# ChaoLiangTHU/rec_now

Measured on AMD Instinct MI355X. Metric: samples/sec fwd+bwd, in-batch pairwise + DCN-v2, B=65536 at 1/2/4/8 GPUs, higher is better.
Workload: dtype f32 via 3 x bf16 six-term split (bf16 MFMA, f32 accumulate; per-product error <= 2^-25)

## Files before the change

rec_now_amd/csrc/gemm_shortk.hip:

```cpp
#include "gemm_split.hpp"

#define SK_BM 128
#define SK_BN 128
#define SK_BK 16

#ifndef RN_SK_PLAIN
#define SK_LDS4(ptr) __builtin_nontemporal_load(reinterpret_cast<const f32x4*>(ptr))
#define SK_STS4(ptr, v) __builtin_nontemporal_store((v), reinterpret_cast<f32x4*>(ptr))
#else
#define SK_LDS4(ptr) (*reinterpret_cast<const f32x4*>(ptr))
#define SK_STS4(ptr, v) (*reinterpret_cast<f32x4*>(ptr) = (v))
#endif
__host__ __device__ constexpr int sk_wg_per_cu(int EP, int DUAL, bool PRE, int NK = 0, bool SPL = false) {
    if (SPL) return 2;
    return (DUAL >= 4 || PRE || (NK > 0 && DUAL == 2)) ? 2 : (EP == 3 || DUAL == 2 || DUAL == 3 || NK > 0) ? 3 : 4;
}

template <bool B_KC, int EP, int DUAL, bool PRE = false, int NK = 0, bool SPL = false>
__global__ void __launch_bounds__(GEMM_THREADS, sk_wg_per_cu(EP, DUAL, PRE, NK, SPL))
k_gemm_shortk(const GemmK p, int row_tiles, int col_tiles, int xcd_aware, const char* __restrict__ b_planes, int64_t b_plane_bytes) {
    static_assert(!SPL || NK >= 3, "split precision: the ring schedule only");
    static_assert(!PRE || ((EP == 1 || EP == 2) && DUAL != 2 && DUAL != 4), "whole-tile prefetch: emul (EP 1) or the old C (EP 2)");
    static_assert(NK % 3 == 0, "ring schedule: three register sets, the same set holds k-tile 0 of every tile");
    static_assert(!PRE || NK == 0 || NK >= 7, "ring schedule: the four groups of the emul tile go out at k-tiles 0, 2, 4, 6");
    using TA = Tile<SK_BM, SK_BK, true>;
    using TB = Tile<SK_BN, SK_BK, B_KC>;
    constexpr int A_SZ = SK_BK * TA::LD, B_SZ = SK_BK * TB::LD, BUF = SPL ? SPL_STAGE / 4 : A_SZ + B_SZ;
    static_assert(4 * 16 * 36 <= BUF, "half sub-tile staging of 4 waves fits one operand buffer");
    extern __shared__ __attribute__((aligned(16))) float smem[];
    const int lane = threadIdx.x & 63, wave = threadIdx.x >> 6;
    const int wm = wave >> 1, wn = wave & 1;
    const int a_off = (lane >> 5) * TA::LD + wm * 64 + (lane & 31);
    const int b_off = (lane >> 5) * TB::LD + wn * 64 + (lane & 31);
    const int col_l = lane & 31, row_l = 4 * (lane >> 5);
    const int rr0 = lane >> 3, cc = (lane & 7) * 4;
    const unsigned e_lane = (unsigned)((wm * 64 + rr0) * p.lde + wn * 64 + cc);
    const unsigned c_lane = (unsigned)((wm * 64 + rr0) * p.ldc + wn * 64 + cc);
    const unsigned f_lane = (unsigned)((wm * 64 + rr0) * p.lde2 + wn * 64 + cc);
    const unsigned d_lane = (unsigned)((wm * 64 + rr0) * p.ldc2 + wn * 64 + cc);
    const unsigned g_lane = (unsigned)((wm * 64 + rr0) * p.lde3 + wn * 64 + cc);
    const int nk = p.K / SK_BK;
    const int ntiles = row_tiles * col_tiles;
    constexpr bool EARLY = NK >= 3 && ((EP && !PRE) || DUAL == 2 || DUAL == 4);
    constexpr bool ONCE = DUAL == 5 || DUAL == 6;
    static_assert(!ONCE || (EP == 0 && NK >= 3), "the one-go input gradient: ring schedule, no emul / accumulate");

    auto tile_of = [&](int slot, int& m0, int& n0) {
        int rt, ct;
        if (xcd_aware) {
            const int xcd = slot & 7, idx = slot >> 3;
            rt = (idx / col_tiles) * 8 + xcd;
            ct = idx % col_tiles;
        } else {
            rt = slot / col_tiles;
            ct = slot % col_tiles;
        }
        m0 = rt * SK_BM;
        n0 = ct * SK_BN;
    };

    TA ta;
    TB tb;
    ta.init(p.lda);
    tb.init(p.ldb);
    int slot = blockIdx.x;
    if (slot >= ntiles) return;
    int m0, n0;
    tile_of(slot, m0, n0);
    f32x4 ra[NK ? 3 : 1][TA::NV], rb[(NK && !SPL) ? 3 : 1][TB::NV];
    u32x4 rp[SPL ? 3 : 1][3];
    unsigned sa_bo = (unsigned)(((threadIdx.x >> 1) * p.lda + 8 * (threadIdx.x & 1)) * 4);
    unsigned sb_bo = (unsigned)((((threadIdx.x >> 7) * p.N) + (threadIdx.x & 127)) * 16);
    const int sa_soff = ((threadIdx.x & 1) * SPL_PLANE_H + (threadIdx.x >> 1)) * 16;
    const int sb_soff = SPL_OPER + ((threadIdx.x >> 7) * SPL_PLANE_H + (threadIdx.x & 127)) * 16;
    const int sfa_off = ((lane >> 5) * SPL_PLANE_H + wm * 64 + (lane & 31)) * 16;
    const int sfb_off = SPL_OPER + ((lane >> 5) * SPL_PLANE_H + wn * 64 + (lane & 31)) * 16;
    auto ring_load = [&](int set, int mm, int nn, int k0) {
        if constexpr (SPL) {
            const char* __restrict__ pa = reinterpret_cast<const char*>(p.A + (int64_t)mm * p.lda + k0);
            const char* __restrict__ pb = b_planes + ((int64_t)(k0 >> 3) * p.N + nn) * 16;
            asm volatile("" : "+v"(sa_bo));
            ra[set][0] = *reinterpret_cast<const f32x4*>(pa + sa_bo);
            ra[set][1] = *reinterpret_cast<const f32x4*>(pa + sa_bo + 16);
            asm volatile("" : "+v"(sb_bo));
#pragma unroll
            for (int q = 0; q < 3; ++q) rp[SPL ? set : 0][q] = *reinterpret_cast<const u32x4*>(pb + q * b_plane_bytes + sb_bo);
        } else {
        const char* __restrict__ pa = reinterpret_cast<const char*>(p.A + TA::tile_base(p.lda, mm, k0));
        const char* __restrict__ pb = reinterpret_cast<const char*>(p.B + TB::tile_base(p.ldb, nn, k0));
#pragma unroll
        for (int i = 0; i < TA::NV; ++i) {
            asm volatile("" : "+v"(ta.boff[i]));
            ra[set][i] = *reinterpret_cast<const f32x4*>(pa + ta.boff[i]);
        }
#pragma unroll
        for (int i = 0; i < TB::NV; ++i) {
            asm volatile("" : "+v"(tb.boff[i]));
            rb[SPL ? 0 : set][i] = *reinterpret_cast<const f32x4*>(pb + tb.boff[i]);
        }
        }
    };
    auto ring_store = [&](int set, float* S) {
        if constexpr (SPL) {
            char* Sc = reinterpret_cast<char*>(S);
            const float x[8] = {ra[set][0].x, ra[set][0].y, ra[set][0].z, ra[set][0].w, ra[set][1].x, ra[set][1].y, ra[set][1].z, ra[set][1].w};
            u32x4 w[3];
            spl_split8(x, w);
#pragma unroll
            for (int q = 0; q < 3; ++q) *reinterpret_cast<u32x4*>(Sc + sa_soff + q * SPL_PLANE) = w[q];
#pragma unroll
            for (int q = 0; q < 3; ++q) *reinterpret_cast<u32x4*>(Sc + sb_soff + q * SPL_PLANE) = rp[SPL ? set : 0][q];
        } else {
#pragma unroll
        for (int i = 0; i < TA::NV; ++i) { ta.v[i] = ra[set][i]; ta.store_slot(i, S); }
#pragma unroll
        for (int i = 0; i < TB::NV; ++i) { tb.v[i] = rb[SPL ? 0 : set][i]; tb.store_slot(i, S + A_SZ); }
        }
    };
    if (NK) {
        ring_load(0, m0, n0, 0);
        ring_load(1, m0, n0, SK_BK);
        ring_store(0, smem);
    } else {
        ta.template load_fast<false>(p.A, nullptr, 0, 0, p.lda, m0, 0);
        tb.template load_fast<false>(p.B, nullptr, 0, 0, p.ldb, n0, 0);
        ta.store(smem);
        tb.store(smem + A_SZ);
    }
    __syncthreads();
    int f = 0;
    for (; slot < ntiles; slot += gridDim.x) {
        const int nslot = slot + gridDim.x;
        const bool has_next = nslot < ntiles;
        int m0n = NK ? m0 : 0, n0n = NK ? n0 : 0;
        if (has_next) tile_of(nslot, m0n, n0n);
#ifdef RN_GEMM_TRACE
#define SK_TR(i) do { if (p.trace && threadIdx.x == 0) p.trace[(long long)slot * 8 + (i)] = wall_clock64(); } while (0)
        if (p.trace && threadIdx.x == 0) {
            p.trace[(long long)slot * 8 + 5] = clock64();
            p.trace[(long long)slot * 8 + 4] = __builtin_amdgcn_s_getreg((4) | (0 << 6) | ((32 - 1) << 11)) |
                                               ((long long)__builtin_amdgcn_s_getreg((20) | (0 << 6) | ((4 - 1) << 11)) << 32);
        }
#else
#define SK_TR(i) do { } while (0)
#endif
        SK_TR(0); SK_TR(1);
        if (p.prio == 1) __builtin_amdgcn_s_setprio(1);
        else if (p.prio == 2) __builtin_amdgcn_s_setprio(2);
        else if (p.prio == 3) __builtin_amdgcn_s_setprio(3);
        f32x16 acc[2][2];
#pragma unroll
        for (int i = 0; i < 2; ++i)
#pragma unroll
            for (int j = 0; j < 2; ++j)
#pragma unroll
                for (int r = 0; r < 16; ++r) acc[i][j][r] = 0.f;
        f32x4 evt[PRE ? 4 : 1][4];
        const float* Etp = !PRE ? nullptr : EP == 1 ? p.emul + (int64_t)m0 * p.lde + n0 : p.C + (int64_t)m0 * p.ldc + n0;
        const int64_t ldp = EP == 1 ? p.lde : p.ldc;
        auto pre_load = [&](int s2) {
#pragma unroll
            for (int q = 0; q < 4; ++q)
                evt[PRE ? s2 : 0][q] = SK_LDS4(Etp + (int64_t)((s2 >> 1) * 32 + q * 8) * ldp + (s2 & 1) * 32 + (EP == 1 ? e_lane : c_lane));
        };
        auto ktile = [&](int cur, int npairs, int nset = -1, float* Sn = nullptr) {
            if constexpr (SPL) {
                const char* S = reinterpret_cast<const char*>(smem + cur * BUF);
                char* Sc = reinterpret_cast<char*>(Sn);
                bf16x8 af[3][2], bf[3][2];
#pragma unroll
                for (int q = 0; q < 3; ++q)
#pragma unroll
                    for (int i = 0; i < 2; ++i) {
                        af[q][i] = *reinterpret_cast<const bf16x8*>(S + q * SPL_PLANE + sfa_off + i * 512);
                        bf[q][i] = *reinterpret_cast<const bf16x8*>(S + q * SPL_PLANE + sfb_off + i * 512);
                    }
                u32x4 w[3];
                const int ns = nset < 0 ? 0 : nset;
                auto pairs = [&](int e0) {
                    const float x[4] = {e0 ? ra[ns][1].x : ra[ns][0].x, e0 ? ra[ns][1].y : ra[ns][0].y, e0 ? ra[ns][1].z : ra[ns][0].z, e0 ? ra[ns][1].w : ra[ns][0].w};
#pragma unroll
                    for (int e = 0; e < 2; ++e) {
                        unsigned p1, p2, p3;
                        spl_split2(x[2 * e], x[2 * e + 1], p1, p2, p3);
                        w[0][e0 + e] = p1; w[1][e0 + e] = p2; w[2][e0 + e] = p3;
                    }
                };
                __builtin_amdgcn_sched_barrier(0);
#define SKS_TERM(SA, SB)                                                                                              \
                _Pragma("unroll") for (int i = 0; i < 2; ++i)                                                         \
                    _Pragma("unroll") for (int j = 0; j < 2; ++j)                                                     \
                        acc[i][j] = __builtin_amdgcn_mfma_f32_32x32x16_bf16(af[SA][i], bf[SB][j], acc[i][j], 0, 0, 0);
                SKS_TERM(0, 0)
                if (nset >= 0) pairs(0);
                __builtin_amdgcn_sched_barrier(0);
                SKS_TERM(0, 1)
                if (nset >= 0) pairs(2);
                __builtin_amdgcn_sched_barrier(0);
                SKS_TERM(1, 0)
                if (nset >= 0) {
#pragma unroll
                    for (int q = 0; q < 3; ++q) *reinterpret_cast<u32x4*>(Sc + sa_soff + q * SPL_PLANE) = w[q];
                }
                __builtin_amdgcn_sched_barrier(0);
                SKS_TERM(1, 1)
                if (nset >= 0) {
#pragma unroll
                    for (int q = 0; q < 3; ++q) *reinterpret_cast<u32x4*>(Sc + sb_soff + q * SPL_PLANE) = rp[SPL ? ns : 0][q];
                }
                __builtin_amdgcn_sched_barrier(0);
                SKS_TERM(0, 2) SKS_TERM(2, 0)
#undef SKS_TERM
                return;
            }
            const float* as = smem + cur * BUF + a_off;
            const float* bs = smem + cur * BUF + A_SZ + b_off;
            float a0[2], b0[2], a1[2], b1[2];
#pragma unroll
            for (int i = 0; i < 2; ++i) a0[i] = FR(as + i * 32);
#pragma unroll
            for (int j = 0; j < 2; ++j) b0[j] = FR(bs + j * 32);
#pragma unroll
            for (int kk = 0; kk < SK_BK; kk += 4) {
#pragma unroll
                for (int i = 0; i < 2; ++i) a1[i] = FR(as + (kk + 2) * TA::LD + i * 32);
#pragma unroll
                for (int j = 0; j < 2; ++j) b1[j] = FR(bs + (kk + 2) * TB::LD + j * 32);
                __builtin_amdgcn_sched_barrier(0);
                if (kk / 2 < npairs) {
#pragma unroll
                    for (int i = 0; i < 2; ++i)
#pragma unroll
                        for (int j = 0; j < 2; ++j) acc[i][j] = __builtin_amdgcn_mfma_f32_32x32x2f32(a0[i], b0[j], acc[i][j], 0, 0, 0);
                }
                __builtin_amdgcn_sched_barrier(0);
                if (kk + 4 < SK_BK) {
#pragma unroll
                    for (int i = 0; i < 2; ++i) a0[i] = FR(as + (kk + 4) * TA::LD + i * 32);
#pragma unroll
                    for (int j = 0; j < 2; ++j) b0[j] = FR(bs + (kk + 4) * TB::LD + j * 32);
                }
                __builtin_amdgcn_sched_barrier(0);
                if (kk / 2 + 1 < npairs) {
#pragma unroll
                    for (int i = 0; i < 2; ++i)
#pragma unroll
                        for (int j = 0; j < 2; ++j) acc[i][j] = __builtin_amdgcn_mfma_f32_32x32x2f32(a1[i], b1[j], acc[i][j], 0, 0, 0);
                }
                __builtin_amdgcn_sched_barrier(0);
            }
        };
        f32x4 ev[2][4], cv[2][4], fv[2][4], dv[2][4];
        float rs[2][4];
        f32x4 hv4[2];
        float hs[4];
        const float* Et = (EP & 1) ? p.emul + (int64_t)m0 * p.lde + n0 : nullptr;
        float* Ct = p.C + (int64_t)m0 * p.ldc + n0;
        const float* Ft = (DUAL == 2 || DUAL == 4) ? p.E2 + (int64_t)m0 * p.lde2 + n0 : nullptr;
        const float* Gt = (DUAL == 4) ? p.E3 + (int64_t)m0 * p.lde3 + n0 : nullptr;
        float* Dt = DUAL ? p.C2 + (int64_t)m0 * p.ldc2 + n0 : nullptr;
        auto issue = [&](int s2, int buf) {
            const int i = s2 >> 1, j = s2 & 1;
#pragma unroll
            for (int q = 0; q < 4; ++q) {
                if ((EP & 1) && !PRE) ev[buf][q] = SK_LDS4(Et + (int64_t)(i * 32 + q * 8) * p.lde + j * 32 + e_lane);
                if ((EP & 2) && !PRE) cv[buf][q] = SK_LDS4(Ct + (int64_t)(i * 32 + q * 8) * p.ldc + j * 32 + c_lane);
                if (DUAL == 2 || DUAL == 4) fv[buf][q] = SK_LDS4(Ft + (int64_t)(i * 32 + q * 8) * p.lde2 + j * 32 + f_lane);
                if (DUAL == 2) dv[buf][q] = SK_LDS4(Dt + (int64_t)(i * 32 + q * 8) * p.ldc2 + j * 32 + d_lane);
                if (DUAL == 4) {
                    dv[buf][q] = SK_LDS4(Gt + (int64_t)(i * 32 + q * 8) * p.lde3 + j * 32 + g_lane);
                    rs[buf][q] = p.rv[m0 + wm * 64 + i * 32 + q * 8 + rr0];
                }
            }
        };
        f32x4 o5[ONCE ? 2 : 1][5][2];
        float r5[ONCE ? 2 : 1][2];
        const float* F1t = ONCE ? p.E2 + (int64_t)m0 * p.lde2 + n0 : nullptr;
        const float* G1t = ONCE ? p.E3 + (int64_t)m0 * p.lde2 + n0 : nullptr;
        const float* F2t = DUAL == 5 ? p.E4 + (int64_t)m0 * p.lde2 + n0 : nullptr;
        const float* G2t = DUAL == 5 ? p.E5 + (int64_t)m0 * p.lde2 + n0 : nullptr;
        const float* H6t = ONCE ? p.E6 + (int64_t)m0 * p.lde2 + n0 : nullptr;
        auto issue5 = [&](int step, int buf) {
            const int s2 = step >> 1, h = step & 1, i = s2 >> 1, j = s2 & 1;
#pragma unroll
            for (int q = 0; q < 2; ++q) {
                const int64_t off = (int64_t)(i * 32 + 16 * h + q * 8) * p.lde2 + j * 32 + f_lane;
                o5[ONCE ? buf : 0][0][q] = SK_LDS4(F1t + off);
                o5[ONCE ? buf : 0][1][q] = SK_LDS4(G1t + off);
                if (DUAL == 5) {
                    o5[ONCE ? buf : 0][2][q] = SK_LDS4(F2t + off);
                    o5[ONCE ? buf : 0][3][q] = SK_LDS4(G2t + off);
                }
                o5[ONCE ? buf : 0][4][q] = SK_LDS4(H6t + off);
                r5[ONCE ? buf : 0][q] = p.rv[m0 + wm * 64 + i * 32 + 16 * h + q * 8 + rr0];
            }
        };
        if (NK) {
#pragma unroll
            for (int t = 0; t < (NK ? NK : 1); ++t) {
                const int cur = (f + t) & 1;
                if (t + 2 < NK) ring_load((t + 2) % 3, m0, n0, (t + 2) * SK_BK);
                else ring_load((t + 2) % 3, m0n, n0n, (t + 2 - NK) * SK_BK);
                if (PRE && (t & 1) == 0 && t < 8) pre_load(t >> 1);
                if (EARLY && t == NK - 3) issue(0, 0);
                if (ONCE && t == NK - 3) issue5(0, 0);
                if constexpr (SPL) {
                    ktile(cur, SK_BK / 2, (t + 1) % 3, smem + (cur ^ 1) * BUF);
                } else {
                    if (t == NK - 1) ktile(cur, p.tail_pairs);
                    else ktile(cur, SK_BK / 2);
                    ring_store((t + 1) % 3, smem + (cur ^ 1) * BUF);
                }
                __syncthreads();
            }
        } else {
            if (PRE) {
#pragma unroll
                for (int s2 = 0; s2 < 4; ++s2) pre_load(s2);
            }
            for (int t = 0; t < nk; ++t) {
                const int cur = (f + t) & 1;
                const bool more = t + 1 < nk;
                if (more) {
                    ta.template load_fast<false>(p.A, nullptr, 0, 0, p.lda, m0, (t + 1) * SK_BK);
                    tb.template load_fast<false>(p.B, nullptr, 0, 0, p.ldb, n0, (t + 1) * SK_BK);
                } else if (has_next) {
                    ta.template load_fast<false>(p.A, nullptr, 0, 0, p.lda, m0n, 0);
                    tb.template load_fast<false>(p.B, nullptr, 0, 0, p.ldb, n0n, 0);
                }
                ktile(cur, (t == nk - 1) ? p.tail_pairs : SK_BK / 2);
                if (more || has_next) {
                    ta.store(smem + (cur ^ 1) * BUF);
                    tb.store(smem + (cur ^ 1) * BUF + A_SZ);
                }
                __syncthreads();
            }
        }
        SK_TR(2);
        if (p.prio) __builtin_amdgcn_s_setprio(0);
        const int fr = (f + nk - 1) & 1;
        float* stg = smem + fr * BUF + wave * (16 * 36);
        if (DUAL == 3 || DUAL == 4 || ONCE) {
            const float* colv = (DUAL == 3 ? p.hv : p.cv) + n0 + wn * 64 + cc;
            hv4[0] = *reinterpret_cast<const f32x4*>(colv);
            hv4[1] = *reinterpret_cast<const f32x4*>(colv + 32);
        }
        if (((EP && !PRE) || DUAL == 2 || DUAL == 4) && !EARLY) issue(0, 0);
#pragma unroll
        for (int s2 = 0; s2 < 4; ++s2) {
            const int i = s2 >> 1, j = s2 & 1, buf = s2 & 1;
            if (((EP && !PRE) || DUAL == 2 || DUAL == 4) && s2 + 1 < 4) issue(s2 + 1, buf ^ 1);
            if (DUAL == 3 && j == 0) hs[0] = hs[1] = hs[2] = hs[3] = 0.f;
#pragma unroll
            for (int h = 0; h < 2; ++h) {
                if (ONCE && 2 * s2 + h + 1 < 8) issue5(2 * s2 + h + 1, (h ^ 1));
#pragma unroll
                for (int r = 0; r < 8; ++r) stg[((r & 3) + 8 * (r >> 2) + row_l) * 36 + col_l] = acc[i][j][8 * h + r];
                RN_LDS_WAVE_SYNC();
#pragma unroll
                for (int q = 0; q < 2; ++q) {
                    const f32x4 a = *reinterpret_cast<const f32x4*>(stg + (q * 8 + rr0) * 36 + cc);
                    f32x4 v = a;
                    if (ONCE) {
                        f32x4 t = (hv4[j] * r5[ONCE ? h : 0][q]) * o5[ONCE ? h : 0][4][q];
                        if (DUAL == 5) t = o5[ONCE ? h : 0][2][q] * o5[ONCE ? h : 0][3][q] + t;
                        t = o5[ONCE ? h : 0][0][q] * o5[ONCE ? h : 0][1][q] + t;
                        v = t + a;
                    }
                    if (EP & 1) v = v * (PRE ? evt[PRE ? s2 : 0][2 * h + q] : ev[buf][2 * h + q]);
                    if (EP & 2) v = v + (PRE ? evt[PRE ? s2 : 0][2 * h + q] : cv[buf][2 * h + q]);
                    if (DUAL != 3) SK_STS4(Ct + (int64_t)(i * 32 + 16 * h + q * 8) * p.ldc + j * 32 + c_lane, v);
                    if (DUAL == 1 || (DUAL == 3 && p.C2 != nullptr)) SK_STS4(Dt + (int64_t)(i * 32 + 16 * h + q * 8) * p.ldc2 + j * 32 + d_lane, a);
                    if (DUAL == 2)
                        *reinterpret_cast<f32x4*>(Dt + (int64_t)(i * 32 + 16 * h + q * 8) * p.ldc2 + j * 32 + d_lane) =
                            dv[buf][2 * h + q] + a * fv[buf][2 * h + q];
                    if (DUAL == 3) {
                        const f32x4 t = v * hv4[j];
                        hs[2 * h + q] += (t.x + t.y) + (t.z + t.w);
                    }
                    if (DUAL == 4)
                        *reinterpret_cast<f32x4*>(Dt + (int64_t)(i * 32 + 16 * h + q * 8) * p.ldc2 + j * 32 + d_lane) =
                            a * fv[buf][2 * h + q] + (hv4[j] * rs[buf][2 * h + q]) * dv[buf][2 * h + q];
                }
                RN_LDS_WAVE_SYNC();
            }
            if (DUAL == 3 && j == 1) {
#pragma unroll
                for (int r = 0; r < 4; ++r) {
                    float t = hs[r];
                    t += __shfl_xor(t, 1, 64);
                    t += __shfl_xor(t, 2, 64);
                    t += __shfl_xor(t, 4, 64);
                    if ((lane & 7) == 0)
                        p.hp[(int64_t)(m0 + wm * 64 + i * 32 + r * 8 + rr0) * p.hp_ld + 2 * (n0 / SK_BN) + wn] = t;
                }
            }
        }
        SK_TR(3);
#ifdef RN_GEMM_TRACE
        if (p.trace && threadIdx.x == 0) p.trace[(long long)slot * 8 + 6] = clock64();
#endif
        __syncthreads();
        f = (f + nk) & 1;
        m0 = m0n;
        n0 = n0n;
    }
}

template <bool B_KC, int EP, int DUAL, bool PRE = false, int NK = 0, bool SPL = false>
static int launch_sk(const GemmK& k, hipStream_t st, const char* planes = nullptr) {
    using TA = Tile<SK_BM, SK_BK, true>;
    using TB = Tile<SK_BN, SK_BK, B_KC>;
    constexpr size_t lds = SPL ? (size_t)2 * SPL_STAGE : 2 * SK_BK * (size_t)(TA::LD + TB::LD) * sizeof(float);
    const int rt = k.M / SK_BM, ct = k.N / SK_BN;
    const int resident = 256 * sk_wg_per_cu(EP, DUAL, PRE, NK, SPL);
    int grid = rt * ct < resident ? rt * ct : resident;
    const int xcd = (rt % 8 == 0 && grid % 8 == 0) ? 1 : 0;
    GemmK kk = k;
    kk.prio = 1;
    const int64_t pb = (int64_t)(k.K / 8) * k.N * 16;
    hipLaunchKernelGGL((k_gemm_shortk<B_KC, EP, DUAL, PRE, NK, SPL>), grid, GEMM_THREADS, lds, st, kk, rt, ct, xcd, planes, pb);
    RN_LAUNCH_CHECK();
    return RECNOW_OK;
}

size_t rn_gemm_shortk_planes_bytes(int K, int N) { return rn_align((size_t)(K / 8) * N * 16 * 3); }

int rn_gemm_launch_shortk_split(const GemmK& k, bool b_kc, int ep, int c2_mode, void* planes, hipStream_t st, const void* ready) {
    if (k.K != 9 * SK_BK || (!planes && !ready) || (int64_t)128 * k.lda >= (1ll << 29)) return RECNOW_EUNSUPPORTED;
    const bool fwd = !b_kc && ep == 1 && (c2_mode == 0 || c2_mode == 1 || c2_mode == 3);
    const bool fwd0 = !b_kc && ep == 0 && c2_mode == 0;
    const bool bwd = b_kc && ((ep == 2 && c2_mode == 0) || (ep == 0 && (c2_mode == 0 || c2_mode == 2 || c2_mode == 4 || c2_mode == 5 || c2_mode == 6)));
    if (!fwd && !fwd0 && !bwd) return RECNOW_EUNSUPPORTED;
    if (!ready) {
        int rc = rn_split_planes(k.B, k.ldb, b_kc ? 1 : 0, k.K, k.N, planes, st);
        if (rc) return rc;
    }
    const char* pl = ready ? (const char*)ready : (const char*)planes;
    if (fwd) {
        if (c2_mode == 1) return launch_sk<false, 1, 1, false, 9, true>(k, st, pl);
        if (c2_mode == 3) return launch_sk<false, 1, 3, false, 9, true>(k, st, pl);
        return launch_sk<false, 1, 0, false, 9, true>(k, st, pl);
    }
    if (fwd0) return launch_sk<false, 0, 0, false, 9, true>(k, st, pl);
    if (ep == 2) return launch_sk<true, 2, 0, false, 9, true>(k, st, pl);
    if (c2_mode == 2) return launch_sk<true, 0, 2, false, 9, true>(k, st, pl);
    if (c2_mode == 4) return launch_sk<true, 0, 4, false, 9, true>(k, st, pl);
    if (c2_mode == 5) return launch_sk<true, 0, 5, false, 9, true>(k, st, pl);
    if (c2_mode == 6) return launch_sk<true, 0, 6, false, 9, true>(k, st, pl);
    return launch_sk<true, 0, 0, false, 9, true>(k, st, pl);
}

int rn_gemm_launch_shortk(const GemmK& k, bool b_kc, int ep, int c2_mode, hipStream_t st) {
    if (k.K == 9 * SK_BK && !b_kc && ep == 1) {
        if (c2_mode == 1) return launch_sk<false, 1, 1, true, 9>(k, st);
        if (c2_mode == 3) return launch_sk<false, 1, 3, true, 9>(k, st);
        if (c2_mode == 0) return launch_sk<false, 1, 0, true, 9>(k, st);
    }
    if (k.K == 9 * SK_BK && !b_kc && ep == 0 && c2_mode == 0) return launch_sk<false, 0, 0, false, 9>(k, st);
    if (k.K == 9 * SK_BK && b_kc && ep == 2 && c2_mode == 0) return launch_sk<true, 2, 0, true, 9>(k, st);
    if (k.K == 9 * SK_BK && b_kc && ep == 0) {
        if (c2_mode == 2) return launch_sk<true, 0, 2, false, 9>(k, st);
        if (c2_mode == 4) return launch_sk<true, 0, 4, false, 9>(k, st);
        if (c2_mode == 5) return launch_sk<true, 0, 5, false, 9>(k, st);
        if (c2_mode == 6) return launch_sk<true, 0, 6, false, 9>(k, st);
        if (c2_mode == 0) return launch_sk<true, 0, 0, false, 9>(k, st);
    }
    if (c2_mode >= 5) return RECNOW_EUNSUPPORTED;
    if (!b_kc && ep == 1) {
        if (c2_mode == 1) return launch_sk<false, 1, 1, true>(k, st);
        if (c2_mode == 3) return launch_sk<false, 1, 3, true>(k, st);
        if (c2_mode == 0) return launch_sk<false, 1, 0, true>(k, st);
    }
    if (c2_mode == 2) return (b_kc && ep == 0) ? launch_sk<true, 0, 2>(k, st) : RECNOW_EUNSUPPORTED;
    if (c2_mode == 4) return (b_kc && ep == 0) ? launch_sk<true, 0, 4>(k, st) : RECNOW_EUNSUPPORTED;
    if (c2_mode) return RECNOW_EUNSUPPORTED;
    if (b_kc) {
        switch (ep) {
            case 0: return launch_sk<true, 0, 0>(k, st);
            case 1: return launch_sk<true, 1, 0>(k, st);
            case 2: return launch_sk<true, 2, 0>(k, st);
            default: return launch_sk<true, 3, 0>(k, st);
        }
    }
    switch (ep) {
        case 0: return launch_sk<false, 0, 0>(k, st);
        case 2: return launch_sk<false, 2, 0>(k, st);
        case 3: return launch_sk<false, 3, 0>(k, st);
        default: return RECNOW_EUNSUPPORTED;
    }
}
```

Measured before the change: 22.92 million.

## Add persistent panel kernel keeping split A row-panel resident in LDS across columns

Adds a 512-thread, one-block-per-CU kernel for the plain-epilogue short-K split GEMM. One group of waves splits a 128-row A panel into three bf16 planes once and keeps them in LDS. Two groups of four waves then walk column tiles in pairs, with a staggered barrier schedule so the groups' phases overlap. This is meant to avoid re-reading and re-splitting A for every output tile, and to overlap the next panel load with the C epilogue. In exchange it uses lower occupancy, large LDS and a delicate barrier-count scheme.

```diff
diff --git a/rec_now_amd/csrc/gemm_shortk.hip b/rec_now_amd/csrc/gemm_shortk.hip
--- a/rec_now_amd/csrc/gemm_shortk.hip
+++ b/rec_now_amd/csrc/gemm_shortk.hip
@@ -1,4 +1,5 @@
 #include "gemm_split.hpp"
+#include <atomic>
 
 #define SK_BM 128
 #define SK_BN 128
@@ -424,6 +425,187 @@
     return RECNOW_OK;
 }
 
+#define SKP_THREADS 512
+#define SKP_HALF (SK_BM * 16)
+#define SKP_KT (3 * 2 * SKP_HALF)
+#define SKP_PANEL (9 * SKP_KT)
+#define SKP_LDS (SKP_PANEL + 4 * SPL_OPER)
+
+__global__ void __launch_bounds__(SKP_THREADS, 1)
+k_gemm_shortk_panel(const GemmK p, int row_tiles, int col_steps, const char* __restrict__ b_planes, int64_t b_plane_bytes) {
+    constexpr int NK = 9;
+    static_assert(4 * 16 * 36 * 4 <= SPL_OPER, "half sub-tile staging of a group's 4 waves fits one weight stage");
+    extern __shared__ __attribute__((aligned(16))) float smem[];
+    char* const panel = reinterpret_cast<char*>(smem);
+    const int lane = threadIdx.x & 63, wave = __builtin_amdgcn_readfirstlane(threadIdx.x >> 6);
+    const int grp = wave >> 2, wv = wave & 3, tg = threadIdx.x & 255;
+    const int wm = wv >> 1, wn = wv & 1;
+    char* const wst = panel + SKP_PANEL + grp * (2 * SPL_OPER);
+    const int col_l = lane & 31, row_l = 4 * (lane >> 5);
+    const int rr0 = lane >> 3, cc = (lane & 7) * 4;
+    const unsigned c_lane = (unsigned)((wm * 64 + rr0) * p.ldc + wn * 64 + cc);
+    unsigned sa_bo = (unsigned)(((tg >> 1) * p.lda + 8 * (tg & 1)) * 4);
+    unsigned sb_bo = (unsigned)((((tg >> 7) * p.N) + (tg & 127)) * 16);
+    const int sa_soff = ((tg & 1) * SK_BM + (tg >> 1)) * 16;
+    const int sb_soff = ((tg >> 7) * SPL_PLANE_H + (tg & 127)) * 16;
+    const int sfa_off = ((lane >> 5) * SK_BM + wm * 64 + (lane & 31)) * 16;
+    const int sfb_off = ((lane >> 5) * SPL_PLANE_H + wn * 64 + (lane & 31)) * 16;
+
+    u32x4 rp[3][3];
+    auto ring_load = [&](int set, int nn, int k0) {
+        const char* __restrict__ pb = b_planes + ((int64_t)(k0 >> 3) * p.N + nn) * 16;
+        asm volatile("" : "+v"(sb_bo));
+#pragma unroll
+        for (int q = 0; q < 3; ++q) rp[set][q] = *reinterpret_cast<const u32x4*>(pb + q * b_plane_bytes + sb_bo);
+    };
+    auto ring_store = [&](int set, char* S) {
+#pragma unroll
+        for (int q = 0; q < 3; ++q) *reinterpret_cast<u32x4*>(S + sb_soff + q * SPL_PLANE) = rp[set][q];
+    };
+    f32x4 pr[NK][2];
+    auto panel_load = [&](int mm) {
+        const char* __restrict__ pa = reinterpret_cast<const char*>(p.A + (int64_t)mm * p.lda);
+        asm volatile("" : "+v"(sa_bo));
+#pragma unroll
+        for (int t = 0; t < NK; ++t) {
+            pr[t][0] = *reinterpret_cast<const f32x4*>(pa + sa_bo + t * (SK_BK * 4));
+            pr[t][1] = *reinterpret_cast<const f32x4*>(pa + sa_bo + t * (SK_BK * 4) + 16);
+        }
+    };
+    auto panel_store = [&]() {
+#pragma unroll
+        for (int t = 0; t < NK; ++t) {
+            const float x[8] = {pr[t][0].x, pr[t][0].y, pr[t][0].z, pr[t][0].w, pr[t][1].x, pr[t][1].y, pr[t][1].z, pr[t][1].w};
+            u32x4 w[3];
+            spl_split8(x, w);
+#pragma unroll
+            for (int q = 0; q < 3; ++q) *reinterpret_cast<u32x4*>(panel + t * SKP_KT + q * (2 * SKP_HALF) + sa_soff) = w[q];
+        }
+    };
+
+    int rt = blockIdx.x;
+    int m0 = rt * SK_BM, n0 = grp * SK_BN;
+    if (grp == 0) panel_load(m0);
+    ring_load(0, n0, 0);
+    ring_load(1, n0, SK_BK);
+    if (grp == 0) panel_store();
+    ring_store(0, wst);
+    __syncthreads();
+    if (grp == 1) {
+#pragma unroll 1
+        for (int b = 0; b < NK; ++b) __syncthreads();
+    }
+    int f = 0;
+    for (; rt < row_tiles; rt += gridDim.x) {
+        const bool next_rt = rt + (int)gridDim.x < row_tiles;
+#pragma unroll 1
+        for (int cs = 0; cs < col_steps; ++cs) {
+            const bool last = cs + 1 == col_steps;
+            const int m0n = last && next_rt ? m0 + (int)gridDim.x * SK_BM : m0;
+            const int n0n = last ? (next_rt ? grp * SK_BN : n0) : n0 + 2 * SK_BN;
+            if (p.prio) __builtin_amdgcn_s_setprio(1);
+            f32x16 acc[2][2];
+#pragma unroll
+            for (int i = 0; i < 2; ++i)
+#pragma unroll
+                for (int j = 0; j < 2; ++j)
+#pragma unroll
+                    for (int r = 0; r < 16; ++r) acc[i][j][r] = 0.f;
+            bf16x8 af[2][3][2], bf[3][2];
+#pragma unroll
+            for (int q = 0; q < 3; ++q)
+#pragma unroll
+                for (int i = 0; i < 2; ++i) af[0][q][i] = *reinterpret_cast<const bf16x8*>(panel + q * (2 * SKP_HALF) + sfa_off + i * 512);
+#pragma unroll
+            for (int t = 0; t < NK; ++t) {
+                const int cur = (f + t) & 1;
+                const char* S = wst + cur * SPL_OPER;
+                if (t + 2 < NK) ring_load((t + 2) % 3, n0, (t + 2) * SK_BK);
+                else ring_load((t + 2) % 3, n0n, (t + 2 - NK) * SK_BK);
+#pragma unroll
+                for (int q = 0; q < 3; ++q)
+#pragma unroll
+                    for (int i = 0; i < 2; ++i) bf[q][i] = *reinterpret_cast<const bf16x8*>(S + q * SPL_PLANE + sfb_off + i * 512);
+                __builtin_amdgcn_sched_barrier(0);
+#define SKP_TERM(SA, SB)                                                                                                      \
+                _Pragma("unroll") for (int i = 0; i < 2; ++i)                                                                 \
+                    _Pragma("unroll") for (int j = 0; j < 2; ++j)                                                             \
+                        acc[i][j] = __builtin_amdgcn_mfma_f32_32x32x16_bf16(af[t & 1][SA][i], bf[SB][j], acc[i][j], 0, 0, 0);
+                SKP_TERM(0, 0)
+                if (t + 1 < NK) {
+#pragma unroll
+                    for (int q = 0; q < 3; ++q)
+#pragma unroll
+                        for (int i = 0; i < 2; ++i)
+                            af[(t + 1) & 1][q][i] = *reinterpret_cast<const bf16x8*>(panel + (t + 1) * SKP_KT + q * (2 * SKP_HALF) + sfa_off + i * 512);
+                }
+                __builtin_amdgcn_sched_barrier(0);
+                SKP_TERM(0, 1)
+                __builtin_amdgcn_sched_barrier(0);
+                SKP_TERM(1, 0)
+                __builtin_amdgcn_sched_barrier(0);
+                SKP_TERM(1, 1)
+                ring_store((t + 1) % 3, wst + (cur ^ 1) * SPL_OPER);
+                __builtin_amdgcn_sched_barrier(0);
+                SKP_TERM(0, 2) SKP_TERM(2, 0)
+#undef SKP_TERM
+                __syncthreads();
+            }
+            if (p.prio) __builtin_amdgcn_s_setprio(0);
+            if (last && next_rt && grp == 1) __syncthreads();
+            if (last && next_rt && grp == 0) panel_load(m0n);
+            float* stg = reinterpret_cast<float*>(wst + ((f + NK - 1) & 1) * SPL_OPER) + wv * (16 * 36);
+            float* Ct = p.C + (int64_t)m0 * p.ldc + n0;
+#pragma unroll
+            for (int s2 = 0; s2 < 4; ++s2) {
+                const int i = s2 >> 1, j = s2 & 1;
+#pragma unroll
+                for (int h = 0; h < 2; ++h) {
+#pragma unroll
+                    for (int r = 0; r < 8; ++r) stg[((r & 3) + 8 * (r >> 2) + row_l) * 36 + col_l] = acc[i][j][8 * h + r];
+                    RN_LDS_WAVE_SYNC();
+#pragma unroll
+                    for (int q = 0; q < 2; ++q) {
+                        const f32x4 a = *reinterpret_cast<const f32x4*>(stg + (q * 8 + rr0) * 36 + cc);
+                        SK_STS4(Ct + (int64_t)(i * 32 + 16 * h + q * 8) * p.ldc + j * 32 + c_lane, a);
+                    }
+                    RN_LDS_WAVE_SYNC();
+                    __syncthreads();
+                }
+            }
+            __syncthreads();
+            if (last && next_rt && grp == 0) {
+                panel_store();
+                __syncthreads();
+            }
+            f ^= 1;
+            m0 = m0n;
+            n0 = n0n;
+        }
+    }
+    if (grp == 0) {
+#pragma unroll 1
+        for (int b = 0; b < NK; ++b) __syncthreads();
+    }
+}
+
+static int launch_skp(const GemmK& k, hipStream_t st, const char* planes) {
+    static std::atomic<bool> raised[64];
+    int dev = 0;
+    RN_HIP(hipGetDevice(&dev));
+    if (dev < 0 || dev >= 64 || !raised[dev].load(std::memory_order_acquire)) {
+        RN_HIP(hipFuncSetAttribute((const void*)k_gemm_shortk_panel, hipFuncAttributeMaxDynamicSharedMemorySize, SKP_LDS));
+        if (dev >= 0 && dev < 64) raised[dev].store(true, std::memory_order_release);
+    }
+    const int rt = k.M / SK_BM;
+    GemmK kk = k;
+    kk.prio = 1;
+    const int64_t pb = (int64_t)(k.K / 8) * k.N * 16;
+    hipLaunchKernelGGL(k_gemm_shortk_panel, rt < 256 ? rt : 256, SKP_THREADS, SKP_LDS, st, kk, rt, k.N / (2 * SK_BN), planes, pb);
+    RN_LAUNCH_CHECK();
+    return RECNOW_OK;
+}
+
 size_t rn_gemm_shortk_planes_bytes(int K, int N) { return rn_align((size_t)(K / 8) * N * 16 * 3); }
 
 int rn_gemm_launch_shortk_split(const GemmK& k, bool b_kc, int ep, int c2_mode, void* planes, hipStream_t st, const void* ready) {
@@ -437,6 +619,7 @@
         if (rc) return rc;
     }
     const char* pl = ready ? (const char*)ready : (const char*)planes;
+    if (ep == 0 && c2_mode == 0 && k.N % (2 * SK_BN) == 0 && k.M >= 2 * SK_BM) return launch_skp(k, st, pl);
     if (fwd) {
         if (c2_mode == 1) return launch_sk<false, 1, 1, false, 9, true>(k, st, pl);
         if (c2_mode == 3) return launch_sk<false, 1, 3, false, 9, true>(k, st, pl);
```

Result: no change. 22.75 million (-0.7%).
